# MechaCritter/Python-Visual-Similarity

Measured on AMD Instinct MI355X. Metric: images/sec encoded + top-k retrieved, VLAD K256 RootSIFT, higher is better.
Workload: dtype f32

## Files before the change

include/pvsim.h:

```cpp
#ifndef PVSIM_H
#define PVSIM_H

#include <stddef.h>
#include <stdint.h>

#ifdef __cplusplus
extern "C" {
#endif

#define PVS_VERSION 103

typedef enum {
  PVS_OK = 0,
  PVS_ERR_INVALID = 1,
  PVS_ERR_NO_DEVICE = 2,
  PVS_ERR_OOM = 3,
  PVS_ERR_UNSUPPORTED = 4,
  PVS_ERR_DIM = 5,
  PVS_ERR_CAPACITY = 6
} pvs_status;

typedef enum {
  PVS_DESC_F32 = 0,
  PVS_DESC_F32_ROOTSIFT = 1,
  PVS_DESC_U8_ROOTSIFT = 2
} pvs_desc_kind;

typedef enum {
  PVS_OPT_ASSIGN_PREFILTER = 0,
  PVS_OPT_VLAD_PATH = 1,
  PVS_OPT_TOPK_SELECT_ONLY = 2,
  PVS_OPT_AGG_VARIANT = 3,
  PVS_OPT_FISHER_SCALE = 4,
  PVS_OPT_TRAIN_BATCH_CHUNKS = 5,
  PVS_OPT_UPDATE_WINDOW_ROWS = 6,
  PVS_OPT_COUNT_ = 7
} pvs_option;

typedef struct pvs_ctx pvs_ctx;
typedef struct pvs_codebook pvs_codebook;
typedef struct pvs_gmm pvs_gmm;
typedef struct pvs_pca pvs_pca;
typedef struct pvs_comm pvs_comm;

typedef struct {
  double power_norm_weight;
  double norm_order;
  double epsilon;
} pvs_norm_params;

int pvs_version(void);
const char* pvs_last_error(void);
int pvs_device_count(int* count);
int pvs_init(int device_id, void* stream, pvs_ctx** out);
int pvs_destroy(pvs_ctx* ctx);
int pvs_sync(pvs_ctx* ctx);
void* pvs_stream(pvs_ctx* ctx);
int pvs_device_name(pvs_ctx* ctx, char* buf, size_t buflen);
int pvs_set_option(pvs_ctx* ctx, int option, int value);
int pvs_get_option(pvs_ctx* ctx, int option, int* value);

int pvs_malloc(pvs_ctx* ctx, size_t bytes, void** dptr);
int pvs_free(pvs_ctx* ctx, void* dptr);
int pvs_memcpy_h2d(pvs_ctx* ctx, void* dst_dev, const void* src_host, size_t bytes);
int pvs_memcpy_d2h(pvs_ctx* ctx, void* dst_host, const void* src_dev, size_t bytes);
int pvs_memset(pvs_ctx* ctx, void* dst_dev, int value, size_t bytes);

int pvs_fill_dev(pvs_ctx* ctx, void* dst_dev, int64_t n_elems, int elem_bytes, uint64_t pattern);
int pvs_stream_wait(pvs_ctx* waiter, pvs_ctx* signal);
// ... 211 lines not shown
```

python-visual-similarity_amd/csrc/common.hpp:

```cpp
#pragma once
#include <hip/hip_runtime.h>

#include <cmath>
#include <cstdarg>
#include <cstdint>
#include <cstdio>
#include <cstring>
#include <map>
#include <type_traits>
#include <vector>

#include "../../include/pvsim.h"
#include "../../include/pvsim_diag.h"
#include "workspace.hpp"

#define PVS_EXPORT extern "C" __attribute__((visibility("default")))

namespace pvs {

void set_error(const char* fmt, ...);

#define PVS_FAIL(code, ...)        \
  do {                             \
    ::pvs::set_error(__VA_ARGS__); \
// ... 17 lines not shown
  } while (0)

#define PVS_NEED(p, what) \
  if (!(p)) PVS_FAIL(PVS_ERR_INVALID, "%s: null %s", __func__, what)
#define PVS_ALIGNED(p, a, what) \
  if (reinterpret_cast<uintptr_t>(p) % (a)) PVS_FAIL(PVS_ERR_INVALID, "%s: %s must be %d-byte aligned", __func__, what, (int)(a))

constexpr int WAVE = 64;

enum TimerSlot { T_ASSIGN = 0, T_AGGREGATE = 1, T_GEMM = 2, T_TOPK = 3, T_FPOST = 4, T_FMOM = 5, T_MISC = 6, T_RESCORE = 7 };

struct TimerRec {
  hipEvent_t a, b;
  int slot;
};

}

struct pvs_ctx {
  int device = 0;
  hipStream_t stream = nullptr;
  bool owns_stream = false;
  int num_cu = 256;
  static constexpr int NWS = 18;
  void* ws[NWS] = {};
  size_t ws_bytes[NWS] = {};
  struct GemmPlanSlot {
    int key[4] = {-1, -1, -1, -1};
    int n_main = 0, n_tail = 0, splitk = 1;
    void* d_tiles = nullptr;
    size_t cap = 0;
  } gemm_plan[5];
  std::map<const void*, int> lds_attr;
  int opt[PVS_OPT_COUNT_] = {1, 0, 0, 0, 0, 0, 0};
  unsigned int* d_queue = nullptr;
  unsigned long long* d_fused_stamps = nullptr;
  bool timers_on = false;
  std::vector<pvs::TimerRec> pending;
  std::vector<hipEvent_t> event_pool;
  std::multimap<size_t, void*> block_cache;
  std::map<void*, size_t> block_size;
  size_t block_cache_bytes = 0;
  void* h_stage = nullptr;
  size_t h_stage_bytes = 0;
  static constexpr int DSIFT_RING = 4;
  void* dsift_h[DSIFT_RING] = {};
  size_t dsift_h_bytes[DSIFT_RING] = {};
  hipEvent_t dsift_ev[DSIFT_RING] = {};
  int dsift_next = 0;
  double t_total[PVS_TIMER_SLOTS] = {0};
  int64_t t_count[PVS_TIMER_SLOTS] = {0};
};

struct pvs_codebook {
  int K = 0, D = 0;
  int K_pad = 0, D_pad = 0;
  float* d_cent = nullptr;
  float* d_cpad = nullptr;
  float* d_cnorm = nullptr;
  void* d_c16 = nullptr;
  int D_pad16 = 0;
  int c16_shift = 0;
  float cmax = 0.f;
  void* d_cnk = nullptr;
  void* d_c16n = nullptr;
  int cn_e1 = 0;
};
// ... 155 lines not shown
```

python-visual-similarity_amd/csrc/cosine.hip:

```cpp
#include <algorithm>
#include <type_traits>

#include "common.hpp"
#include "gemm_mfma.hpp"
#include "gemm_f64.hpp"
#include "gemm_f16_8ph.hpp"
#include "gemm_f16_2lvl.hpp"

namespace pvs {

__device__ __attribute__((aligned(16))) float g_zero16[4] = {0.f, 0.f, 0.f, 0.f};

__global__ __launch_bounds__(256) void row_inv_norms_kernel(const float* __restrict__ x, int64_t rows, int64_t L,
                                                            float* __restrict__ inv, int vec) {
  const int lane = threadIdx.x & 63;
  const int64_t row = (int64_t)blockIdx.x * 4 + (threadIdx.x >> 6);
  if (row >= rows) return;
  const float* p = x + row * L;
  float s0 = 0.f, s1 = 0.f, s2 = 0.f, s3 = 0.f;
  if (vec) {
    const float4* p4 = reinterpret_cast<const float4*>(p);
    for (int64_t i = lane; i < (L >> 2); i += 64) {
      const float4 v = p4[i];
      s0 = fmaf(v.x, v.x, s0); s1 = fmaf(v.y, v.y, s1); s2 = fmaf(v.z, v.z, s2); s3 = fmaf(v.w, v.w, s3);
// ... 52 lines not shown
    const int full = total / slots, rem = total % slots;
    double best = rounds(total);
    P.n_main = total;
    P.n_tail = 0;
    P.splitk = 1;
    for (int sk = 2; sk <= 32; sk *= 2) {
      if (rem > 0) {
        const double a = full + rounds((long)rem * sk) * (1.0 / sk + eps) + red * rem;
        if (a < best - 1e-9) { best = a; P.n_main = total - rem; P.n_tail = rem; P.splitk = sk; }
      }
      if (total < 4 * slots) {
        const double b = rounds((long)total * sk) * (1.0 / sk + eps) + red * total;
        if (b < best - 1e-9) { best = b; P.n_main = 0; P.n_tail = total; P.splitk = sk; }
      }
    }
    if (P.cap < t.size()) {
      PVS_HIP(hipStreamSynchronize(ctx->stream));
      if (P.d_tiles) PVS_HIP(hipFree(P.d_tiles));
      P.d_tiles = nullptr;
      P.cap = 0;
      P.key[0] = -1;
      const size_t cap = t.size() + t.size() / 4 + 64;
      PVS_HIP(hipMalloc(&P.d_tiles, cap * sizeof(GemmTile)));
      P.cap = cap;
    }
    PVS_HIP(hipMemcpyAsync(P.d_tiles, t.data(), t.size() * sizeof(GemmTile), hipMemcpyHostToDevice, ctx->stream));
    PVS_HIP(hipStreamSynchronize(ctx->stream));
    memcpy(P.key, key, sizeof(key));
  }
  *out = &P;
  return PVS_OK;
}

template <bool SYMM, int MODEL, bool DUAL = false>
static int launch_gemm_mfma(pvs_ctx* ctx, GemmArgs g, const GemmPlan& plan) {
  using GM = GemmModel<MODEL>;
  using Cfg = typename GM::Cfg;
  constexpr bool F16 = GM::F16;
  constexpr int BM = GM::BM, WM = 2, WN = GM::WN;
  constexpr bool TWO = GM::TWO, ILV = MODEL == 1 && !SYMM;
  auto kfull = gemm_mfma_kernel<BM, BM, WM, WN, 2, SYMM, 2, GEMM_MODE_FULL, false, F16, TWO, ILV, DUAL>;
  auto kpart = gemm_mfma_kernel<BM, BM, WM, WN, 2, SYMM, 2, GEMM_MODE_PARTIAL, false, F16, TWO, ILV, DUAL>;
  auto kred = gemm_mfma_kernel<BM, BM, WM, WN, 2, SYMM, 2, GEMM_MODE_REDUCE, false, F16, TWO, ILV, DUAL>;
  for (const void* k : {reinterpret_cast<const void*>(kfull), reinterpret_cast<const void*>(kpart),
                        reinterpret_cast<const void*>(kred)})
    PVS_TRY(ensure_lds(ctx, k, Cfg::LDS_BYTES));
  if (plan.n_main > 0) {
    g.tile_base = 0;
    if constexpr (MODEL == 1) {
      auto k8 = gemm_f16_8ph_kernel<SYMM, true>;
      PVS_TRY(ensure_lds(ctx, reinterpret_cast<const void*>(k8), G8_LDS_BYTES));
      hipLaunchKernelGGL(k8, dim3((unsigned)plan.n_main), dim3(512), G8_LDS_BYTES, ctx->stream, g);
    } else {
      hipLaunchKernelGGL(kfull, dim3((unsigned)plan.n_main), dim3(Cfg::THREADS), Cfg::LDS_BYTES, ctx->stream, g);
    }
  }
  if (plan.n_tail > 0) {
    const int bk = F16 ? 64 : 32;
    const int nk = (int)((g.L + bk - 1) / bk);
    const int nparts = TWO ? (nk + GEMM_KBLOCK / bk - 1) / (GEMM_KBLOCK / bk) : plan.splitk;
    const size_t bytes = (size_t)plan.n_tail * nparts * BM * BM * sizeof(float);
    if (bytes > ((size_t)1 << 30)) {
      g.tile_base = plan.n_main;
      hipLaunchKernelGGL(kfull, dim3((unsigned)plan.n_tail), dim3(Cfg::THREADS), Cfg::LDS_BYTES, ctx->stream, g);
    } else {
      float* part = nullptr;
      PVS_TRY(ws_reserve(ctx, WS_AUX_ROWS, bytes, &part));
      g.tile_base = plan.n_main;
      g.splitk = std::min(plan.splitk, nparts);
      g.nparts = nparts;
      g.partial = part;
      hipLaunchKernelGGL(kpart, dim3((unsigned)(plan.n_tail * g.splitk)), dim3(Cfg::THREADS), Cfg::LDS_BYTES, ctx->stream, g);
      hipLaunchKernelGGL(kred, dim3((unsigned)plan.n_tail), dim3(Cfg::THREADS), Cfg::LDS_BYTES, ctx->stream, g);
    }
  }
// ... 3 lines not shown

template <int MODEL>
static int cosine_mfma(pvs_ctx* ctx, const void* A, int64_t M, const void* B, int64_t N, int64_t L, const float* inva,
                       const float* invb, float* out, int64_t ldo, float* out_t = nullptr, int64_t ldt = 0, int64_t ld = 0,
                       int accumulate = 0) {
  constexpr int BT = GemmModel<MODEL>::BM;
  const int tiles_m = (int)((M + BT - 1) / BT), tiles_n = (int)((N + BT - 1) / BT);
  if ((int64_t)tiles_m * tiles_n > 0x3fffffffLL) PVS_FAIL(PVS_ERR_UNSUPPORTED, "cosine: too many tiles for one launch");
  const bool symm = (A == B) && (M == N) && (inva == invb) && out_t == nullptr;
  GemmPlan* plan = nullptr;
  if constexpr (MODEL == 2) {
    const int t256 = (int)((M + 255) / 256), t128 = (int)((N + 127) / 128);
    if (!symm && out_t == nullptr && (int64_t)t256 * t128 >= (int64_t)4 * ctx->num_cu && (int64_t)t256 * t128 <= 0x3fffffffLL &&
        L <= (int64_t)8 * 1024 * 1024) {
      PVS_TRY(build_plan(ctx, 4, t256, t128, false, ctx->num_cu, &plan));
      GemmArgs g{};
      g.A = A; g.B = B; g.M = M; g.N = N; g.L = L; g.lda = ld ? ld : L; g.ldb = ld ? ld : L; g.inva = inva; g.invb = invb;
      g.accumulate = accumulate;
      g.out = out; g.ldo = ldo; g.tiles = static_cast<const GemmTile*>(plan->d_tiles); g.splitk = 1; g.tile_base = 0;
      PVS_HIP(hipGetSymbolAddress(reinterpret_cast<void**>(const_cast<float**>(&g.zero16)), HIP_SYMBOL(g_zero16)));
      auto k2 = gemm_f16_2lvl_kernel<false>;
      PVS_TRY(ensure_lds(ctx, reinterpret_cast<const void*>(k2), G2_LDS_BYTES));
      hipLaunchKernelGGL(k2, dim3((unsigned)(plan->n_main + plan->n_tail)), dim3(512), G2_LDS_BYTES, ctx->stream, g);
      PVS_HIP(hipGetLastError());
      return PVS_OK;
    }
  }
  PVS_TRY(build_plan(ctx, MODEL, tiles_m, tiles_n, symm, ctx->num_cu * GemmModel<MODEL>::PER_CU, &plan));
  GemmArgs g{};
  g.A = A; g.B = B; g.M = M; g.N = N; g.L = L; g.lda = ld ? ld : L; g.ldb = ld ? ld : L; g.inva = inva; g.invb = invb;
  g.accumulate = accumulate;
  g.out = out; g.ldo = ldo; g.out_t = out_t; g.ldt = ldt; g.tiles = static_cast<const GemmTile*>(plan->d_tiles); g.splitk = 1;
  PVS_HIP(hipGetSymbolAddress(reinterpret_cast<void**>(const_cast<float**>(&g.zero16)), HIP_SYMBOL(g_zero16)));
  if (symm) return launch_gemm_mfma<true, MODEL>(ctx, g, *plan);
  if constexpr (MODEL == 0) {
    if (out_t) return launch_gemm_mfma<false, 0, true>(ctx, g, *plan);
  }
  return launch_gemm_mfma<false, MODEL>(ctx, g, *plan);
}

__global__ __launch_bounds__(256) void f32_to_f16_kernel(const float4* __restrict__ src, int64_t n4, uint2* __restrict__ dst) {
  for (int64_t i = (int64_t)blockIdx.x * blockDim.x + threadIdx.x; i < n4; i += (int64_t)gridDim.x * blockDim.x) {
    const float4 v = src[i];
    union { _Float16 h[4]; uint2 u; } o;
    o.h[0] = (_Float16)v.x; o.h[1] = (_Float16)v.y; o.h[2] = (_Float16)v.z; o.h[3] = (_Float16)v.w;
    dst[i] = o.u;
  }
}
__global__ void f32_to_f16_tail_kernel(const float* __restrict__ src, int64_t start, int64_t n, _Float16* __restrict__ dst) {
  const int64_t i = start + (int64_t)blockIdx.x * blockDim.x + threadIdx.x;
  if (i < n) dst[i] = (_Float16)src[i];
}

int launch_f32_to_f16(pvs_ctx* ctx, const float* src, int64_t n, void* dst) {
  if (n <= 0) return PVS_OK;
  ScopedTimer tm(ctx, T_MISC);
  const bool vec = reinterpret_cast<uintptr_t>(src) % 16 == 0 && reinterpret_cast<uintptr_t>(dst) % 8 == 0;
  const int64_t n4 = vec ? n / 4 : 0;
  if (n4 > 0) {
    const unsigned grid = (unsigned)std::min<int64_t>((n4 + 255) / 256, (int64_t)ctx->num_cu * 16);
    hipLaunchKernelGGL(f32_to_f16_kernel, dim3(grid), dim3(256), 0, ctx->stream, reinterpret_cast<const float4*>(src), n4,
                       reinterpret_cast<uint2*>(dst));
  }
  if (n4 * 4 < n)
    hipLaunchKernelGGL(f32_to_f16_tail_kernel, dim3((unsigned)((n - n4 * 4 + 255) / 256)), dim3(256), 0, ctx->stream, src,
                       n4 * 4, n, reinterpret_cast<_Float16*>(dst));
  PVS_HIP(hipGetLastError());
  return PVS_OK;
}

// ... 186 lines not shown
```

python-visual-similarity_amd/csrc/gemm_mfma.hpp:

```cpp
#pragma once
#include <hip/hip_runtime.h>

#include <cstdint>

namespace pvs {

typedef float f32x16_t __attribute__((ext_vector_type(16)));
typedef float f32x4_t __attribute__((ext_vector_type(4)));

struct GemmTile {
  int tm, tn;
};

struct GemmArgs {
  const void* A;
  const void* B;
  int64_t M, N, L;
  int64_t lda, ldb;
  const float* inva;
  const float* invb;
  float* out;
  int64_t ldo;
  float* out_t;
  int64_t ldt;
  const GemmTile* tiles;
  int tile_base;
  int splitk;
  int nparts;
  float* partial;
  const float* zero16;
  unsigned long long* stamps;
  int accumulate;
  int dbg;
};

#ifndef PVS_GEMM_DBG
// ... 160 lines not shown
    const unsigned m0a = lds0 + s0 * RING_UNIT_BYTES + wave_off, m0b = lds0 + s1 * RING_UNIT_BYTES + wave_off;
    constexpr int U = IS_A ? 0 : 2;
    asm volatile("s_mov_b32 m0, %0\n\ts_nop 0\n\t"
                 "global_load_lds_dwordx4 %3, %2\n\t"
                 "global_load_lds_dwordx4 %4, %2 offset:1024\n\t"
                 "s_mov_b32 m0, %1\n\ts_nop 0\n\t"
                 "global_load_lds_dwordx4 %5, %2\n\t"
                 "global_load_lds_dwordx4 %6, %2 offset:1024"
                 ::"s"(m0a), "s"(m0b), "s"(sb), "v"(voff[U][0]), "v"(voff[U][1]), "v"(voff[U + 1][0]), "v"(voff[U + 1][1])
                 : "memory");
  }
  template <bool IS_A>
  __device__ __forceinline__ void issue_checked(const GemmArgs& g, int64_t k0, char* smem, int s0, int s1) const {
    constexpr int U = IS_A ? 0 : 2;
#pragma unroll
    for (int u = 0; u < 2; ++u)
#pragma unroll
      for (int q = 0; q < 2; ++q) {
        const char* p = (k0 + gce[q] < g.L) ? (IS_A ? base_a : base_b) + k0 * 2 + (size_t)voff[U + u][q] + q * 1024
                                         : reinterpret_cast<const char*>(g.zero16);
        __builtin_amdgcn_global_load_lds((const __attribute__((address_space(1))) void*)p,
                                         (__attribute__((address_space(3))) void*)(smem + (u ? s1 : s0) * RING_UNIT_BYTES + wave_off + q * 1024),
                                         16, 0, 0);
      }
  }
};

template <int IMM>
__device__ __forceinline__ void ds_read_frag_imm(f32x4_t& dst, unsigned addr) {
  asm volatile("ds_read_b128 %0, %1 offset:%2" : "=v"(dst) : "v"(addr), "n"(IMM));
}

template <int BM, int BN, int WM, int WN, int STAGES, bool SYMM, int OCC, int MODE = GEMM_MODE_FULL, bool STAMP = false,
          bool F16 = false, bool TWO = true, bool ILV = false, bool DUAL = false, int LW = WM * WN, bool PP = false>
__global__ __launch_bounds__(64 * WM * WN, OCC) void gemm_mfma_kernel(GemmArgs g) {
  using Cfg = GemmCfg<BM, BN, WM, WN, STAGES, F16, LW>;
  constexpr int GEMM_BK = Cfg::BK;
  constexpr int MI = Cfg::MI, NI = Cfg::NI;
  static_assert(!(SYMM || DUAL) || BM == BN, "the mirrored store needs square tiles");
  static_assert(!(SYMM && DUAL), "SYMM already mirrors");
  extern __shared__ __attribute__((aligned(16))) char smem[];
  const int lane = threadIdx.x & 63;
  const int wave = __builtin_amdgcn_readfirstlane(threadIdx.x >> 6);
  const int i = lane & 31, h = lane >> 5;
  const int wm = wave / WN, wn = wave % WN;

  int lin, slice = 0;
  {
    int bid = blockIdx.x;
    if constexpr (MODE == GEMM_MODE_PARTIAL) {
      slice = bid % g.splitk;
      bid /= g.splitk;
    }
    if constexpr (MODE == GEMM_MODE_FULL) {
      const int nwg = gridDim.x;
      const int xcd = bid & 7, pos = bid >> 3;
      const int q8 = nwg >> 3, r8 = nwg & 7;
      lin = (xcd < r8 ? xcd * (q8 + 1) : r8 * (q8 + 1) + (xcd - r8) * q8) + pos;
    } else {
      lin = bid;
    }
  }
  const GemmTile tile = g.tiles[g.tile_base + lin];
  const int tm = tile.tm, tn = tile.tn;
  const int64_t m0 = (int64_t)tm * BM, n0 = (int64_t)tn * BN;

  f32x16_t acc[MI][NI];
// ... 7 lines not shown
  if constexpr (MODE != GEMM_MODE_REDUCE) {
    f32x16_t tot[TWO ? MI : 1][TWO ? NI : 1];
    if constexpr (TWO) {
#pragma unroll
      for (int a = 0; a < MI; ++a)
#pragma unroll
        for (int b = 0; b < NI; ++b)
#pragma unroll
          for (int r = 0; r < 16; ++r) tot[a][b][r] = 0.f;
    }

    const int nk_all = (int)((g.L + GEMM_BK - 1) / GEMM_BK);
    constexpr int CHAIN_KT = GEMM_KBLOCK / GEMM_BK;
    int kt0 = 0, kt1 = nk_all;
    if constexpr (MODE == GEMM_MODE_PARTIAL) {
      const int unit = TWO ? CHAIN_KT : 1;
      const int units = (nk_all + unit - 1) / unit;
      const int per = ((units + g.splitk - 1) / g.splitk) * unit;
      kt0 = min(nk_all, slice * per);
      kt1 = min(nk_all, kt0 + per);
    }
    const bool ktail = (g.L % GEMM_BK) != 0;
    GemmLoader<Cfg> ld;
    const bool loader = wave < Cfg::LOADER_WAVES;
    if (loader && !PP) ld.init(g, m0, n0, wave, lane);
    auto stage_tile = [&](int t) {
      if (!loader) return;
      char* st = smem + ((t - kt0) % STAGES) * Cfg::STAGE_BYTES;
      if (ktail && t == nk_all - 1) ld.issue_checked(g, (int64_t)t * GEMM_BK, st);
      else ld.template issue<0, Cfg::LOADS_PER_WAVE>((int64_t)t * GEMM_BK, st);
    };
    if constexpr (!PP) {
#pragma unroll
      for (int s = 0; s < STAGES - 1; ++s)
        if (kt0 + s < kt1) stage_tile(kt0 + s);
    }

    unsigned offa[MI][4], offb[NI][4];
#pragma unroll
    for (int t = 0; t < 4; ++t) {
#pragma unroll
      for (int a = 0; a < MI; ++a) offa[a][t] = gemm_frag_off(wm * (32 * MI) + 32 * a + i, 2 * t + h);
#pragma unroll
      for (int b = 0; b < NI; ++b) offb[b][t] = Cfg::A_BYTES + gemm_frag_off(wn * (32 * NI) + 32 * b + i, 2 * t + h);
    }
    const unsigned lds0 = lds_addr(smem);
    unsigned long long st_t0 = 0, st_r0 = 0, seg[4] = {0, 0, 0, 0};
    if constexpr (STAMP) {
      st_t0 = __builtin_amdgcn_s_memtime();
      st_r0 = __builtin_amdgcn_s_memrealtime();
    }

    if constexpr (PP) {
      static_assert(F16 && !TWO && !ILV && STAGES == 2 && WM == 2 && WN == 4 && BM == 256 && BN == 256 && LW == 8,
                    "ping-pong: fp16, 256 x 256, eight waves");
      const bool g1 = wm != 0;
      constexpr bool DBG = STAMP || PVS_GEMM_DBG;
      const int dbg = DBG ? g.dbg : 0;
      GemmRingLoader rl;
      rl.init(g, (dbg & 8) ? 0 : m0, (dbg & 8) ? 0 : n0, wave, lane);
      const int T = kt1 - kt0;
      auto load = [&](int u, bool is_a) {
        const int kt = kt0 + u;
        const int j = 4 * u + (is_a ? 0 : 2);
        const int s0 = j % RING_UNITS, s1 = (j + 1) % RING_UNITS;
        const int64_t k0 = (int64_t)kt * GEMM_BK;
        if (ktail && kt == nk_all - 1) {
          if (is_a) rl.issue_checked<true>(g, k0, smem, s0, s1);
          else rl.issue_checked<false>(g, k0, smem, s0, s1);
        } else {
          if (is_a) rl.issue<true>(k0, lds0, s0, s1);
          else rl.issue<false>(k0, lds0, s0, s1);
        }
      };
      unsigned fo[4];
#pragma unroll
      for (int t = 0; t < 4; ++t) fo[t] = 128 * i + 16 * ((2 * t + h) ^ ((i >> 1) & 7));
      const unsigned b_half = (wn & 1) * 8192;
      if (T > 0) { load(0, true); load(0, false); }
      if (T > 1) { load(1, true); wait_vm<4>(); } else wait_vm<0>();
      __builtin_amdgcn_s_barrier();
      if (g1) __builtin_amdgcn_s_barrier();
      f32x4_t av[2][MI], bv[2][NI];
      for (int u = 0; u < T; ++u) {
// ... 34 lines not shown
                                                                   __builtin_bit_cast(f16x8_t, bv[s2][b]), acc[a][b], 0, 0, 0);
          __builtin_amdgcn_s_setprio(0);
          __builtin_amdgcn_sched_barrier(0);
        };
        unsigned long long p0 = 0, p1 = 0, p2 = 0, p3 = 0, p4 = 0, p5 = 0, p6 = 0, p7 = 0, p8 = 0;
        if constexpr (STAMP) p0 = __builtin_amdgcn_s_memtime();
        if (g1) issue_b();
        reads(0);
        if constexpr (STAMP) p1 = __builtin_amdgcn_s_memtime();
        __builtin_amdgcn_s_barrier();
        if constexpr (STAMP) p2 = __builtin_amdgcn_s_memtime();
        if (!g1) issue_b();
        mfmas();
        if constexpr (STAMP) p3 = __builtin_amdgcn_s_memtime();
        __builtin_amdgcn_s_barrier();
        if constexpr (STAMP) p4 = __builtin_amdgcn_s_memtime();
        if (g1) issue_a();
        reads(1);
        if (g1) landed();
        if constexpr (STAMP) p5 = __builtin_amdgcn_s_memtime();
        __builtin_amdgcn_s_barrier();
        if constexpr (STAMP) p6 = __builtin_amdgcn_s_memtime();
        if (!g1) issue_a();
        mfmas();
        if (!g1) landed();
        if constexpr (STAMP) p7 = __builtin_amdgcn_s_memtime();
        __builtin_amdgcn_s_barrier();
        if constexpr (STAMP) {
          p8 = __builtin_amdgcn_s_memtime();
          seg[0] += (p1 - p0) + (p5 - p4); seg[1] += (p2 - p1) + (p6 - p5); seg[2] += (p3 - p2) + (p7 - p6); seg[3] += (p4 - p3) + (p8 - p7);
        }
      }
      if (!g1) __builtin_amdgcn_s_barrier();
    } else
    for (int kt = kt0; kt < kt1; ++kt) {
      unsigned long long s0 = 0, s1 = 0, s2 = 0, s3 = 0;
      if constexpr (STAMP) s0 = __builtin_amdgcn_s_memtime();
      if (kt + STAGES - 2 < kt1) wait_vm<(STAGES - 2) * Cfg::LOADS_PER_WAVE>();
      else wait_vm<0>();
      if constexpr (STAMP) s1 = __builtin_amdgcn_s_memtime();
      __builtin_amdgcn_s_barrier();
      if constexpr (STAMP) s2 = __builtin_amdgcn_s_memtime();
      const int tnext = kt + STAGES - 1;
      const bool inl = ILV && tnext < kt1 && !(ktail && tnext == nk_all - 1);
      if (tnext < kt1 && !inl) stage_tile(tnext);
      if constexpr (STAMP) s3 = __builtin_amdgcn_s_memtime();
      const unsigned base = lds0 + ((kt - kt0) % STAGES) * Cfg::STAGE_BYTES;
      f32x4_t av[2][MI], bv[2][NI];
#pragma unroll
      for (int a = 0; a < MI; ++a) ds_read_frag(av[0][a], base + offa[a][0]);
#pragma unroll
      for (int b = 0; b < NI; ++b) ds_read_frag(bv[0][b], base + offb[b][0]);
#pragma unroll
      for (int t = 0; t < 4; ++t) {
        const int c = t & 1, n = c ^ 1;
        if (t < 3) {
#pragma unroll
          for (int a = 0; a < MI; ++a) ds_read_frag(av[n][a], base + offa[a][t + 1]);
#pragma unroll
          for (int b = 0; b < NI; ++b) ds_read_frag(bv[n][b], base + offb[b][t + 1]);
        }
        if constexpr (ILV) {
          if (inl && loader) {
            constexpr int QN = Cfg::LOADS_PER_WAVE;
            char* st = smem + ((tnext - kt0) % STAGES) * Cfg::STAGE_BYTES;
            const int64_t k0n = (int64_t)tnext * GEMM_BK;
// ... 1 lines not shown
            if (t == 1) ld.template issue<QN / 4, QN / 2>(k0n, st);
            if (t == 2) ld.template issue<QN / 2, 3 * QN / 4>(k0n, st);
            if (t == 3) ld.template issue<3 * QN / 4, QN>(k0n, st);
          }
        }
        if (t < 3) wait_lgkm<MI + NI>();
        else wait_lgkm<0>();
        __builtin_amdgcn_sched_barrier(0);
        if constexpr (F16) {
          if constexpr (F16_PRIO) __builtin_amdgcn_s_setprio(1);
#pragma unroll
          for (int a = 0; a < MI; ++a)
#pragma unroll
            for (int b = 0; b < NI; ++b)
              acc[a][b] = __builtin_amdgcn_mfma_f32_32x32x16_f16(__builtin_bit_cast(f16x8_t, av[c][a]),
                                                                 __builtin_bit_cast(f16x8_t, bv[c][b]), acc[a][b], 0, 0, 0);
          if constexpr (F16_PRIO) __builtin_amdgcn_s_setprio(0);
        } else {
#pragma unroll
          for (int e = 0; e < 4; ++e) {
#pragma unroll
            for (int a = 0; a < MI; ++a)
#pragma unroll
              for (int b = 0; b < NI; ++b)
                acc[a][b] = __builtin_amdgcn_mfma_f32_32x32x2f32(av[c][a][e], bv[c][b][e], acc[a][b], 0, 0, 0);
          }
        }
        __builtin_amdgcn_sched_barrier(0);
      }
      if constexpr (STAMP) {
        const unsigned long long s4 = __builtin_amdgcn_s_memtime();
        seg[0] += s1 - s0; seg[1] += s2 - s1; seg[2] += s3 - s2; seg[3] += s4 - s3;
      }
      if constexpr (TWO) {
        if ((kt & (CHAIN_KT - 1)) == CHAIN_KT - 1 || (MODE == GEMM_MODE_PARTIAL && kt == kt1 - 1)) {
          if constexpr (MODE == GEMM_MODE_PARTIAL) {
            float* dst = g.partial + ((int64_t)lin * g.nparts + kt / CHAIN_KT) * (BM * BN) + wave * (MI * NI * 1024);
#pragma unroll
            for (int a = 0; a < MI; ++a)
#pragma unroll
              for (int b = 0; b < NI; ++b)
#pragma unroll
                for (int r = 0; r < 16; ++r) {
                  dst[(a * NI + b) * 1024 + r * 64 + lane] = acc[a][b][r];
                  acc[a][b][r] = 0.f;
                }
          } else {
#pragma unroll
            for (int a = 0; a < MI; ++a)
#pragma unroll
              for (int b = 0; b < NI; ++b) {
                tot[a][b] += acc[a][b];
#pragma unroll
                for (int r = 0; r < 16; ++r) acc[a][b][r] = 0.f;
              }
          }
        }
      }
    }
    if constexpr (STAMP) {
      const unsigned long long t1 = __builtin_amdgcn_s_memtime(), r1 = __builtin_amdgcn_s_memrealtime();
      if (threadIdx.x == 0 && g.stamps) {
        unsigned long long* o = g.stamps + 8 * blockIdx.x;
        o[0] = st_t0; o[1] = t1; o[2] = st_r0; o[3] = r1;
        o[4] = seg[0]; o[5] = seg[1]; o[6] = seg[2]; o[7] = seg[3];
      }
    }
    if constexpr (TWO) {
#pragma unroll
      for (int a = 0; a < MI; ++a)
#pragma unroll
        for (int b = 0; b < NI; ++b) acc[a][b] += tot[a][b];
    }
  }

  constexpr int PART_ELEMS = BM * BN;
  if constexpr (MODE == GEMM_MODE_PARTIAL) {
    if constexpr (!TWO) {
      float* dst = g.partial + ((int64_t)lin * g.nparts + slice) * PART_ELEMS + wave * (MI * NI * 1024);
#pragma unroll
      for (int a = 0; a < MI; ++a)
#pragma unroll
        for (int b = 0; b < NI; ++b)
#pragma unroll
          for (int r = 0; r < 16; ++r) dst[(a * NI + b) * 1024 + r * 64 + lane] = acc[a][b][r];
    }
    return;
  }
  if constexpr (MODE == GEMM_MODE_REDUCE) {
    for (int s = 0; s < g.nparts; ++s) {
      const float* src = g.partial + ((int64_t)lin * g.nparts + s) * PART_ELEMS + wave * (MI * NI * 1024);
#pragma unroll
      for (int a = 0; a < MI; ++a)
#pragma unroll
        for (int b = 0; b < NI; ++b)
#pragma unroll
          for (int r = 0; r < 16; ++r) acc[a][b][r] += src[(a * NI + b) * 1024 + r * 64 + lane];
    }
// ... 47 lines not shown
```

python-visual-similarity_amd/pvsim/_ffi.py:

```python
from __future__ import annotations

import ctypes as C
import os
import threading

import numpy as np

from ._errors import CapacityError

_HERE = os.path.dirname(os.path.abspath(__file__))
LIB_PATH = os.environ.get("PVSIM_LIB", os.path.join(_HERE, "libpvsim_hip.so"))

PVS_OK, PVS_ERR_INVALID, PVS_ERR_NO_DEVICE, PVS_ERR_OOM, PVS_ERR_UNSUPPORTED, PVS_ERR_DIM, PVS_ERR_CAPACITY = range(7)
_EXC = {PVS_ERR_INVALID: ValueError, PVS_ERR_NO_DEVICE: RuntimeError, PVS_ERR_OOM: MemoryError,
        PVS_ERR_UNSUPPORTED: NotImplementedError, PVS_ERR_DIM: RuntimeError, PVS_ERR_CAPACITY: CapacityError}

DESC_F32, DESC_F32_ROOTSIFT, DESC_U8_ROOTSIFT = 0, 1, 2
OPT_ASSIGN_PREFILTER, OPT_VLAD_PATH, OPT_TOPK_SELECT_ONLY, OPT_AGG_VARIANT, OPT_FISHER_SCALE = 0, 1, 2, 3, 4
OPT_TRAIN_BATCH_CHUNKS = 5
PIX_U8_RGB, PIX_U8_GRAY, PIX_F32_RGB, PIX_F32_GRAY = 0, 1, 2, 3
DSIFT_U8, DSIFT_F32, DSIFT_F32_RAW, DSIFT_F32_QUANT = 0, 1, 2, 3
OPT_UPDATE_WINDOW_ROWS = 6
SCAN_TILE = 2048
COMBINE_CHUNK_BYTES, COMBINE_BATCH = 8192, 8
DIFFUSE_DOT_BLOCK, DIFFUSE_MAX_COLUMNS = 256, 65536
VLAD_PATH_AUTO, VLAD_PATH_GATHER, VLAD_PATH_STREAM, VLAD_PATH_FUSED = 0, 1, 2, 3
TIMER_NAMES = ("assign", "aggregate", "cosine_gemm", "topk", "fisher_posterior", "fisher_moments", "misc", "rescore")


class NormParams(C.Structure):
    _fields_ = [("power_norm_weight", C.c_double), ("norm_order", C.c_double), ("epsilon", C.c_double)]


_vp, _i64, _int, _sz = C.c_void_p, C.c_int64, C.c_int, C.c_size_t
_pp = C.POINTER(C.c_void_p)
_np = C.POINTER(NormParams)

SIGNATURES = {
    "pvs_version": [],
    "pvs_last_error": [],
    "pvs_device_count": [C.POINTER(C.c_int)],
    "pvs_init": [_int, _vp, _pp],
    "pvs_destroy": [_vp],
    "pvs_sync": [_vp],
    "pvs_stream": [_vp],
    "pvs_device_name": [_vp, C.c_char_p, _sz],
    "pvs_set_option": [_vp, _int, _int],
    "pvs_get_option": [_vp, _int, C.POINTER(C.c_int)],
    "pvs_malloc": [_vp, _sz, _pp],
    "pvs_free": [_vp, _vp],
    "pvs_memcpy_h2d": [_vp, _vp, _vp, _sz],
    "pvs_memcpy_d2h": [_vp, _vp, _vp, _sz],
    "pvs_memset": [_vp, _vp, _int, _sz],
    "pvs_fill_dev": [_vp, _vp, _i64, _int, C.c_uint64],
    "pvs_stream_wait": [_vp, _vp],
# ... 167 lines not shown
```

python-visual-similarity_amd/pvsim/engine.py:

```python
from __future__ import annotations

import ctypes as C
import os
import sys
import threading

import numpy as np

from . import _ffi
from ._ffi import DESC_F32, DESC_F32_ROOTSIFT, DESC_U8_ROOTSIFT, check, norm_params, ptr

__all__ = ["Context", "default_context", "pack_descriptors", "dsift_count", "dsift_frames", "sift_workspace", "diffuse_workspace", "DESC_F32", "DESC_F32_ROOTSIFT", "DESC_U8_ROOTSIFT"]


def pack_descriptors(desc_list, dim: int, dtype=np.float32):
    counts = [0 if d is None else int(d.shape[0]) for d in desc_list]
    offsets = np.zeros(len(desc_list) + 1, dtype=np.int64)
    np.cumsum(counts, out=offsets[1:])
    packed = np.empty((int(offsets[-1]), dim), dtype=dtype)
    for d, o in zip(desc_list, offsets[:-1]):
        if d is not None and d.shape[0]:
            if d.shape[1] != dim:
                raise RuntimeError(f"descriptor dimension {d.shape[1]} does not match the model input dimension {dim}")
            packed[o:o + d.shape[0]] = d
# ... 92 lines not shown

    def download(self, shape, dtype, offset: int = 0) -> np.ndarray:
        out = np.empty(shape, dtype=dtype)
        if offset + out.nbytes > self.nbytes:
            raise ValueError("download past the end of the device buffer")
        check(_ffi.lib().pvs_memcpy_d2h(self._ctx.handle, ptr(out), C.c_void_p(self.ptr + offset), out.nbytes))
        return out

    def fill_bytes(self, value: int):
        check(_ffi.lib().pvs_memset(self._ctx.handle, C.c_void_p(self.ptr), int(value), self.nbytes))
        return self

    def free(self):
        if self.ptr and not getattr(self, "_borrowed", False) and self._ctx.handle is not None:
            if not self._ctx._give_cached(self.ptr, getattr(self, "_cap", self.nbytes)):
                _ffi.lib().pvs_free(self._ctx.handle, C.c_void_p(self.ptr))
        self.ptr = 0

    def __del__(self):
        try:
            self.free()
        except Exception:
            pass


class Context:

    def __init__(self, device: int = 0, stream: int | None = None):
        self.handle = None
        h = C.c_void_p()
        check(_ffi.lib().pvs_init(int(device), C.c_void_p(stream), C.byref(h)))
        self.handle = h
        self.device = int(device)
        self._cache = []

    _CACHE_BLOCKS, _CACHE_BYTES = 24, 2 << 30

    def _take_cached(self, nbytes):
        best = None
        for i, (cap, p) in enumerate(self._cache):
            if nbytes <= cap <= 2 * nbytes + 4096 and (best is None or cap < self._cache[best][0]):
                best = i
        if best is None:
            return None
        cap, p = self._cache.pop(best)
        return p, cap

    def _give_cached(self, p, cap):
        if len(self._cache) >= self._CACHE_BLOCKS or cap + sum(c for c, _ in self._cache) > self._CACHE_BYTES:
            return False
        self._cache.append((int(cap), int(p)))
        return True

    def trim(self):
        while self._cache:
            _, p = self._cache.pop()
            if self.handle is not None:
                _ffi.lib().pvs_free(self.handle, C.c_void_p(p))

    def close(self):
        if self.handle is not None:
            self.trim()
            _ffi.lib().pvs_destroy(self.handle)
            self.handle = None

    def __del__(self):
# ... 533 lines not shown
```

Measured before the change: 409,300.

## Add rotated fp32 MFMA k-loop that moves the barrier to the tile hand-over

Adds a ROT variant of the fp32 MFMA GEMM k-loop that prefetches all stages up front, double-buffers LDS fragment reads across sub-steps, and places the workgroup barrier and next-tile global stage at the end of each k-tile, overlapping with the next fragment reads. The goal is to cut barrier stalls at the top of each k-tile and keep the MFMA pipe busier in the cosine GEMM. The variant becomes the default for MODEL 0 through a new option, and the old schedule stays reachable via an environment variable. It adds register pressure from the doubled fragment buffers and a profiling helper script.

Measured after the change: 411,600 (median of 6 runs). No clear change (+0.6%).

```diff
diff --git a/include/pvsim.h b/include/pvsim.h
--- a/include/pvsim.h
+++ b/include/pvsim.h
@@ -34,7 +34,8 @@
   PVS_OPT_FISHER_SCALE = 4,
   PVS_OPT_TRAIN_BATCH_CHUNKS = 5,
   PVS_OPT_UPDATE_WINDOW_ROWS = 6,
-  PVS_OPT_COUNT_ = 7
+  PVS_OPT_GEMM_SCHEDULE = 7,
+  PVS_OPT_COUNT_ = 8
 } pvs_option;
 
 typedef struct pvs_ctx pvs_ctx;
diff --git a/profiles/gemm_schedule_summarize.py b/profiles/gemm_schedule_summarize.py
--- /dev/null
+++ b/profiles/gemm_schedule_summarize.py
@@ -0,0 +1,70 @@
+#!/usr/bin/env python3
+import collections, csv, glob, json, statistics, sys
+
+NAMES = {1: "parent: barrier at the top of the k-tile", 0: "rotated hand-over (default)"}
+
+
+def tag(sched, run, session):
+    d = json.loads(sys.stdin.read().strip().splitlines()[-1])
+    g = d["stages"]["cosine_gemm"]
+    print(json.dumps({"session": session, "gemm_schedule": sched, "schedule": NAMES[sched], "run": run, "ms_per_step": d["ms_per_step"],
+                      "cosine_gemm_ms": round(g["ms_total"] / d["steps"], 4), "value": d["value"], "unit": d["unit"],
+                      "stages_ms_per_step": {k: round(v["ms_total"] / d["steps"], 4) for k, v in d["stages"].items()},
+                      "roofline_achieved_TFLOPs": d["roofline"]["achieved"], "device": d["device"],
+                      "command": "PVSIM_GEMM_SCHEDULE=%d python3 bench.py --gpus 1 --steps 20 --warmup 5 --no-cpu-baseline" % sched}))
+
+
+def verdict(path):
+    allrows = [json.loads(l) for l in open(path) if l.strip()]
+    for session in sorted({r["session"] for r in allrows}):
+        rows = [r for r in allrows if r["session"] == session]
+        res = {"session": session}
+        for key in ("cosine_gemm_ms", "ms_per_step"):
+            p = [r[key] for r in rows if r["gemm_schedule"] == 1]
+            c = [r[key] for r in rows if r["gemm_schedule"] == 0]
+            spread = max(p) - min(p)
+            diff = statistics.median(p) - statistics.median(c)
+            res[key] = {"parent": p, "rotated": c, "parent_spread": round(spread, 4), "median_gain_ms": round(diff, 4),
+                        "slowest_rotated_below_fastest_parent": max(c) < min(p), "gain_over_3x_spread": diff > 3 * spread}
+        print(json.dumps(res))
+
+
+def pmc(src, dst):
+    out = {"command": "PVSIM_GEMM_SCHEDULE=s rocprofv3 --kernel-trace --stats | --pmc SQ_VALU_MFMA_BUSY_CYCLES SQ_BUSY_CU_CYCLES "
+                      "(passes of their own) --output-format csv -- python3 bench.py --gpus 1 --steps 20 --warmup 5 --no-cpu-baseline",
+           "note": "fp32 gemm_mfma_kernel launches only; `main` = the full-round launch (grid 2048), the split-K tail is listed apart"}
+    for sched in (1, 0):
+        rec = {}
+        hits = glob.glob(f"{src}/mfma{sched}/**/*_counter_collection.csv", recursive=True)
+        if hits:
+            acc = collections.defaultdict(lambda: collections.defaultdict(float))
+            for r in csv.DictReader(open(hits[0])):
+                nm = r["Kernel_Name"]
+                if "pvs::gemm_mfma_kernel" in nm:
+                    acc[nm.split("(")[0].replace("void ", "")][r["Counter_Name"]] += float(r["Counter_Value"])
+            for k, d in acc.items():
+                if d.get("SQ_BUSY_CU_CYCLES"):
+                    rec.setdefault(k, {})["mfma_pipe_busy_frac"] = round(d["SQ_VALU_MFMA_BUSY_CYCLES"] / (4.0 * d["SQ_BUSY_CU_CYCLES"]), 4)
+        hits = glob.glob(f"{src}/stats{sched}/**/*_kernel_trace.csv", recursive=True)
+        if hits:
+            dur = collections.defaultdict(list)
+            for r in csv.DictReader(open(hits[0])):
+                nm = r["Kernel_Name"]
+                if "pvs::gemm_mfma_kernel" in nm:
+                    dur[nm.split("(")[0].replace("void ", "")].append((int(r["End_Timestamp"]) - int(r["Start_Timestamp"])) * 1e-6)
+            for k, v in dur.items():
+                v.sort()
+                rec.setdefault(k, {})["launch_ms"] = {"n": len(v), "min": round(v[0], 4), "median": round(v[len(v) // 2], 4),
+                                                      "max": round(v[-1], 4), "mean": round(sum(v) / len(v), 4)}
+        out[NAMES[sched]] = rec
+    json.dump(out, open(dst, "w"), indent=1)
+    print(json.dumps(out))
+
+
+if __name__ == "__main__":
+    if sys.argv[1] == "tag":
+        tag(int(sys.argv[2]), int(sys.argv[3]), int(sys.argv[4]) if len(sys.argv) > 4 else 1)
+    elif sys.argv[1] == "verdict":
+        verdict(sys.argv[2])
+    elif sys.argv[1] == "pmc":
+        pmc(sys.argv[2], sys.argv[3])
diff --git a/python-visual-similarity_amd/csrc/common.hpp b/python-visual-similarity_amd/csrc/common.hpp
--- a/python-visual-similarity_amd/csrc/common.hpp
+++ b/python-visual-similarity_amd/csrc/common.hpp
@@ -73,7 +73,7 @@
     size_t cap = 0;
   } gemm_plan[5];
   std::map<const void*, int> lds_attr;
-  int opt[PVS_OPT_COUNT_] = {1, 0, 0, 0, 0, 0, 0};
+  int opt[PVS_OPT_COUNT_] = {1, 0, 0, 0, 0, 0, 0, 0};
   unsigned int* d_queue = nullptr;
   unsigned long long* d_fused_stamps = nullptr;
   bool timers_on = false;
diff --git a/python-visual-similarity_amd/csrc/cosine.hip b/python-visual-similarity_amd/csrc/cosine.hip
--- a/python-visual-similarity_amd/csrc/cosine.hip
+++ b/python-visual-similarity_amd/csrc/cosine.hip
@@ -108,15 +108,15 @@
   return PVS_OK;
 }
 
-template <bool SYMM, int MODEL, bool DUAL = false>
+template <bool SYMM, int MODEL, bool DUAL = false, bool ROT = false>
 static int launch_gemm_mfma(pvs_ctx* ctx, GemmArgs g, const GemmPlan& plan) {
   using GM = GemmModel<MODEL>;
   using Cfg = typename GM::Cfg;
   constexpr bool F16 = GM::F16;
   constexpr int BM = GM::BM, WM = 2, WN = GM::WN;
   constexpr bool TWO = GM::TWO, ILV = MODEL == 1 && !SYMM;
-  auto kfull = gemm_mfma_kernel<BM, BM, WM, WN, 2, SYMM, 2, GEMM_MODE_FULL, false, F16, TWO, ILV, DUAL>;
-  auto kpart = gemm_mfma_kernel<BM, BM, WM, WN, 2, SYMM, 2, GEMM_MODE_PARTIAL, false, F16, TWO, ILV, DUAL>;
+  auto kfull = gemm_mfma_kernel<BM, BM, WM, WN, 2, SYMM, 2, GEMM_MODE_FULL, false, F16, TWO, ILV, DUAL, WM * WN, false, ROT>;
+  auto kpart = gemm_mfma_kernel<BM, BM, WM, WN, 2, SYMM, 2, GEMM_MODE_PARTIAL, false, F16, TWO, ILV, DUAL, WM * WN, false, ROT>;
   auto kred = gemm_mfma_kernel<BM, BM, WM, WN, 2, SYMM, 2, GEMM_MODE_REDUCE, false, F16, TWO, ILV, DUAL>;
   for (const void* k : {reinterpret_cast<const void*>(kfull), reinterpret_cast<const void*>(kpart),
                         reinterpret_cast<const void*>(kred)})
@@ -186,10 +186,15 @@
   g.accumulate = accumulate;
   g.out = out; g.ldo = ldo; g.out_t = out_t; g.ldt = ldt; g.tiles = static_cast<const GemmTile*>(plan->d_tiles); g.splitk = 1;
   PVS_HIP(hipGetSymbolAddress(reinterpret_cast<void**>(const_cast<float**>(&g.zero16)), HIP_SYMBOL(g_zero16)));
+  if constexpr (MODEL == 0) {
+    if (ctx->opt[PVS_OPT_GEMM_SCHEDULE] == 0) {
+      if (symm) return launch_gemm_mfma<true, 0, false, true>(ctx, g, *plan);
+      if (out_t) return launch_gemm_mfma<false, 0, true, true>(ctx, g, *plan);
+      return launch_gemm_mfma<false, 0, false, true>(ctx, g, *plan);
+    }
+    if (out_t) return launch_gemm_mfma<false, 0, true>(ctx, g, *plan);
+  }
   if (symm) return launch_gemm_mfma<true, MODEL>(ctx, g, *plan);
-  if constexpr (MODEL == 0) {
-    if (out_t) return launch_gemm_mfma<false, 0, true>(ctx, g, *plan);
-  }
   return launch_gemm_mfma<false, MODEL>(ctx, g, *plan);
 }
 
diff --git a/python-visual-similarity_amd/csrc/gemm_mfma.hpp b/python-visual-similarity_amd/csrc/gemm_mfma.hpp
--- a/python-visual-similarity_amd/csrc/gemm_mfma.hpp
+++ b/python-visual-similarity_amd/csrc/gemm_mfma.hpp
@@ -2,6 +2,7 @@
 #include <hip/hip_runtime.h>
 
 #include <cstdint>
+#include <type_traits>
 
 namespace pvs {
 
@@ -228,7 +229,8 @@
 }
 
 template <int BM, int BN, int WM, int WN, int STAGES, bool SYMM, int OCC, int MODE = GEMM_MODE_FULL, bool STAMP = false,
-          bool F16 = false, bool TWO = true, bool ILV = false, bool DUAL = false, int LW = WM * WN, bool PP = false>
+          bool F16 = false, bool TWO = true, bool ILV = false, bool DUAL = false, int LW = WM * WN, bool PP = false,
+          bool ROT = false>
 __global__ __launch_bounds__(64 * WM * WN, OCC) void gemm_mfma_kernel(GemmArgs g) {
   using Cfg = GemmCfg<BM, BN, WM, WN, STAGES, F16, LW>;
   constexpr int GEMM_BK = Cfg::BK;
@@ -302,7 +304,7 @@
     };
     if constexpr (!PP) {
 #pragma unroll
-      for (int s = 0; s < STAGES - 1; ++s)
+      for (int s = 0; s < (ROT ? STAGES : STAGES - 1); ++s)
         if (kt0 + s < kt1) stage_tile(kt0 + s);
     }
 
@@ -320,6 +322,35 @@
       st_t0 = __builtin_amdgcn_s_memtime();
       st_r0 = __builtin_amdgcn_s_memrealtime();
     }
+    auto chain_cut = [&](int kt) {
+      if constexpr (TWO) {
+        if ((kt & (CHAIN_KT - 1)) == CHAIN_KT - 1 || (MODE == GEMM_MODE_PARTIAL && kt == kt1 - 1)) {
+          if constexpr (MODE == GEMM_MODE_PARTIAL) {
+            float* dst = g.partial + ((int64_t)lin * g.nparts + kt / CHAIN_KT) * (BM * BN) + wave * (MI * NI * 1024);
+#pragma unroll
+            for (int a = 0; a < MI; ++a)
+#pragma unroll
+              for (int b = 0; b < NI; ++b)
+#pragma unroll
+                for (int r = 0; r < 16; ++r) {
+                  dst[(a * NI + b) * 1024 + r * 64 + lane] = acc[a][b][r];
+                  acc[a][b][r] = 0.f;
+                }
+          } else {
+#pragma unroll
+            for (int a = 0; a < MI; ++a)
+#pragma unroll
+              for (int b = 0; b < NI; ++b) {
+                tot[a][b] += acc[a][b];
+#pragma unroll
+                for (int r = 0; r < 16; ++r) acc[a][b][r] = 0.f;
+              }
+          }
+        }
+      }
+    };
+    unsigned hw_id = 0;
+    if constexpr (STAMP) hw_id = __builtin_amdgcn_s_getreg((15 << 11) | 4);
 
     if constexpr (PP) {
       static_assert(F16 && !TWO && !ILV && STAGES == 2 && WM == 2 && WN == 4 && BM == 256 && BN == 256 && LW == 8,
@@ -420,6 +451,78 @@
         }
       }
       if (!g1) __builtin_amdgcn_s_barrier();
+    } else if constexpr (ROT) {
+      static_assert(!F16 && !ILV && STAGES == 2, "rotated k-loop: exact fp32, two stages, burst issue");
+      f32x4_t av[2][MI], bv[2][NI];
+      unsigned fa[MI][4], fb[NI][4];
+#pragma unroll
+      for (int t = 0; t < 4; ++t) {
+#pragma unroll
+        for (int a = 0; a < MI; ++a) fa[a][t] = lds0 + offa[a][t];
+#pragma unroll
+        for (int b = 0; b < NI; ++b) fb[b][t] = lds0 + offb[b][t];
+      }
+      if (kt0 < kt1) {
+        if (kt0 + 1 < kt1) wait_vm<Cfg::LOADS_PER_WAVE>();
+        else wait_vm<0>();
+        __builtin_amdgcn_s_barrier();
+#pragma unroll
+        for (int a = 0; a < MI; ++a) ds_read_frag_imm<0>(av[0][a], fa[a][0]);
+#pragma unroll
+        for (int b = 0; b < NI; ++b) ds_read_frag_imm<0>(bv[0][b], fb[b][0]);
+      }
+      auto tile = [&](auto buf, int kt) {
+        constexpr int CUR = decltype(buf)::value * Cfg::STAGE_BYTES, NXT = (decltype(buf)::value ^ 1) * Cfg::STAGE_BYTES;
+        unsigned long long s0 = 0, s1 = 0, s2 = 0, s3 = 0, s4 = 0;
+        if constexpr (STAMP) s0 = __builtin_amdgcn_s_memtime();
+#pragma unroll
+        for (int t = 0; t < 4; ++t) {
+          const int c = t & 1, n = c ^ 1;
+          if (t < 3) {
+#pragma unroll
+            for (int a = 0; a < MI; ++a) ds_read_frag_imm<CUR>(av[n][a], fa[a][t + 1]);
+#pragma unroll
+            for (int b = 0; b < NI; ++b) ds_read_frag_imm<CUR>(bv[n][b], fb[b][t + 1]);
+            wait_lgkm<MI + NI>();
+          } else {
+            if constexpr (STAMP) s1 = __builtin_amdgcn_s_memtime();
+            wait_lgkm<0>();
+            if (kt + 1 < kt1) {
+              wait_vm<0>();
+              if constexpr (STAMP) s2 = __builtin_amdgcn_s_memtime();
+              __builtin_amdgcn_s_barrier();
+              if constexpr (STAMP) s3 = __builtin_amdgcn_s_memtime();
+              if (kt + 2 < kt1) stage_tile(kt + 2);
+#pragma unroll
+              for (int a = 0; a < MI; ++a) ds_read_frag_imm<NXT>(av[0][a], fa[a][0]);
+#pragma unroll
+              for (int b = 0; b < NI; ++b) ds_read_frag_imm<NXT>(bv[0][b], fb[b][0]);
+            } else if constexpr (STAMP) {
+              s2 = s3 = s1;
+            }
+            if constexpr (STAMP) s4 = __builtin_amdgcn_s_memtime();
+          }
+          __builtin_amdgcn_sched_barrier(0);
+#pragma unroll
+          for (int e = 0; e < 4; ++e) {
+#pragma unroll
+            for (int a = 0; a < MI; ++a)
+#pragma unroll
+              for (int b = 0; b < NI; ++b)
+                acc[a][b] = __builtin_amdgcn_mfma_f32_32x32x2f32(av[c][a][e], bv[c][b][e], acc[a][b], 0, 0, 0);
+          }
+          __builtin_amdgcn_sched_barrier(0);
+        }
+        if constexpr (STAMP) {
+          const unsigned long long s5 = __builtin_amdgcn_s_memtime();
+          seg[0] += s2 - s1; seg[1] += s3 - s2; seg[2] += s4 - s3; seg[3] += (s1 - s0) + (s5 - s4);
+        }
+        chain_cut(kt);
+      };
+      for (int kt = kt0; kt < kt1; kt += 2) {
+        tile(std::integral_constant<int, 0>{}, kt);
+        if (kt + 1 < kt1) tile(std::integral_constant<int, 1>{}, kt + 1);
+      }
     } else
     for (int kt = kt0; kt < kt1; ++kt) {
       unsigned long long s0 = 0, s1 = 0, s2 = 0, s3 = 0;
@@ -487,31 +590,7 @@
         const unsigned long long s4 = __builtin_amdgcn_s_memtime();
         seg[0] += s1 - s0; seg[1] += s2 - s1; seg[2] += s3 - s2; seg[3] += s4 - s3;
       }
-      if constexpr (TWO) {
-        if ((kt & (CHAIN_KT - 1)) == CHAIN_KT - 1 || (MODE == GEMM_MODE_PARTIAL && kt == kt1 - 1)) {
-          if constexpr (MODE == GEMM_MODE_PARTIAL) {
-            float* dst = g.partial + ((int64_t)lin * g.nparts + kt / CHAIN_KT) * (BM * BN) + wave * (MI * NI * 1024);
-#pragma unroll
-            for (int a = 0; a < MI; ++a)
-#pragma unroll
-              for (int b = 0; b < NI; ++b)
-#pragma unroll
-                for (int r = 0; r < 16; ++r) {
-                  dst[(a * NI + b) * 1024 + r * 64 + lane] = acc[a][b][r];
-                  acc[a][b][r] = 0.f;
-                }
-          } else {
-#pragma unroll
-            for (int a = 0; a < MI; ++a)
-#pragma unroll
-              for (int b = 0; b < NI; ++b) {
-                tot[a][b] += acc[a][b];
-#pragma unroll
-                for (int r = 0; r < 16; ++r) acc[a][b][r] = 0.f;
-              }
-          }
-        }
-      }
+      chain_cut(kt);
     }
     if constexpr (STAMP) {
       const unsigned long long t1 = __builtin_amdgcn_s_memtime(), r1 = __builtin_amdgcn_s_memrealtime();
@@ -519,6 +598,10 @@
         unsigned long long* o = g.stamps + 8 * blockIdx.x;
         o[0] = st_t0; o[1] = t1; o[2] = st_r0; o[3] = r1;
         o[4] = seg[0]; o[5] = seg[1]; o[6] = seg[2]; o[7] = seg[3];
+        {
+          o[4] |= (unsigned long long)hw_id << 48;
+          o[5] |= (unsigned long long)(__builtin_amdgcn_s_getreg((3 << 11) | 20) & 15u) << 48;
+        }
       }
     }
     if constexpr (TWO) {
diff --git a/python-visual-similarity_amd/pvsim/_ffi.py b/python-visual-similarity_amd/pvsim/_ffi.py
--- a/python-visual-similarity_amd/pvsim/_ffi.py
+++ b/python-visual-similarity_amd/pvsim/_ffi.py
@@ -21,6 +21,7 @@
 PIX_U8_RGB, PIX_U8_GRAY, PIX_F32_RGB, PIX_F32_GRAY = 0, 1, 2, 3
 DSIFT_U8, DSIFT_F32, DSIFT_F32_RAW, DSIFT_F32_QUANT = 0, 1, 2, 3
 OPT_UPDATE_WINDOW_ROWS = 6
+OPT_GEMM_SCHEDULE = 7
 SCAN_TILE = 2048
 COMBINE_CHUNK_BYTES, COMBINE_BATCH = 8192, 8
 DIFFUSE_DOT_BLOCK, DIFFUSE_MAX_COLUMNS = 256, 65536
diff --git a/python-visual-similarity_amd/pvsim/engine.py b/python-visual-similarity_amd/pvsim/engine.py
--- a/python-visual-similarity_amd/pvsim/engine.py
+++ b/python-visual-similarity_amd/pvsim/engine.py
@@ -148,6 +148,8 @@
         check(_ffi.lib().pvs_init(int(device), C.c_void_p(stream), C.byref(h)))
         self.handle = h
         self.device = int(device)
+        if os.environ.get("PVSIM_GEMM_SCHEDULE") in ("0", "1"):
+            self.set_option(_ffi.OPT_GEMM_SCHEDULE, int(os.environ["PVSIM_GEMM_SCHEDULE"]))
         self._cache = []
 
     _CACHE_BLOCKS, _CACHE_BYTES = 24, 2 << 30
```
